# mythos-bio/mythos

Hardware: AMD Instinct MI355X
Metric: MD steps/sec (and ns/day) per GPU, oxDNA2 12 kbp duplex (higher is better)
Workload: dtype f32; 1 GPU; oxDNA2 12000 bp duplex (24000 nt), Debye-Hueckel salt 0.5, Langevin dt 0.005, free space, 1 replica/GPU; half_charged_ends=True, replicas=1, repeats=1, warmup_steps_done=10205, precision=headline f32 (north_star: fp32 at 1e-3); the other precision: --full, full=False

## Files before the change

include/mythos_hip.h:

```cpp
#ifndef MYTHOS_HIP_H
#define MYTHOS_HIP_H

#include <stdint.h>

#ifdef __cplusplus
extern "C" {
#endif

typedef struct mythos_system mythos_system_t;
typedef struct mythos_sim mythos_sim_t;
typedef struct mythos_martini mythos_martini_t;
typedef struct mythos_martini_sim mythos_martini_sim_t;
typedef struct mythos_obs mythos_obs_t;
typedef void* mythos_stream_t;

enum mythos_status {
  MYTHOS_OK = 0,
  MYTHOS_ERR_INVALID_ARGUMENT = -1,
  MYTHOS_ERR_HIP = -2,
  MYTHOS_ERR_NO_DEVICE = -3,
  MYTHOS_ERR_NOT_READY = -4,
  MYTHOS_ERR_OVERFLOW = -5,
  MYTHOS_ERR_NUMERIC = -6
};

enum mythos_dtype { MYTHOS_F32 = 0, MYTHOS_F64 = 1 };

#define MYTHOS_OXDNA_N_TERMS 8

const char* mythos_version(void);
const char* mythos_last_error(void);
int mythos_device_count(void);

int mythos_oxdna_param_count(void);
const char* mythos_oxdna_param_name(int index);

mythos_system_t* mythos_oxdna_create(int model, int n, const int32_t* seq, const uint8_t* is_end, int n_bonded,
                                     const int32_t* bonded, const double* box, int dtype, int device);
void mythos_oxdna_destroy(mythos_system_t* sys);

int mythos_oxdna_set_params(mythos_system_t* sys, const double* flat_params, int n_params);

int mythos_oxdna_set_nucleotide_types(mythos_system_t* sys, const uint8_t* is_rna);

int mythos_oxdna_set_pseq(mythos_system_t* sys, const double* marginals, const int32_t* unit, int n_bp,
                          const double* bp_probs, int terms);

int mythos_oxdna_energy_dpseq(mythos_system_t* sys, const void* center, const void* quat, int n_frames, double* e_terms,
                              void* dU_dcenter, void* dU_dquat, double* dU_dparams, double* dU_dmarginals, double* dU_dbp,
                              mythos_stream_t stream);

int mythos_oxdna_set_neighbors(mythos_system_t* sys, const int32_t* pairs, int n_pairs);

int mythos_oxdna_build_neighbors(mythos_system_t* sys, const void* center, double r_cut, double skin,
                                 mythos_stream_t stream);
int mythos_oxdna_neighbor_stats(mythos_system_t* sys, int* max_row, double* mean_row);

int mythos_oxdna_energy(mythos_system_t* sys, const void* center, const void* quat, int n_frames, double* e_terms,
                        void* dU_dcenter, void* dU_dquat, double* dU_dparams, mythos_stream_t stream);

#define MYTHOS_DEBYE_SWEEP_CONSTS 5
int mythos_oxdna_debye_sweep(mythos_system_t* sys, const void* center, const void* quat, int n_frames, int n_kt,
                             const double* dh_consts, double* e_dh, double* de_dconsts, mythos_stream_t stream);

#define MYTHOS_OP_BOND 0
#define MYTHOS_OP_MINDISTANCE 1
int mythos_oxdna_order_params(mythos_system_t* sys, const void* center, const void* quat, int n_frames, int n_ops,
                              const int32_t* op_kind, const int32_t* op_first, const int32_t* pairs, int n_pairs,
                              double hb_cutoff, double* op_out, double* hb_out, double* dist_out, mythos_stream_t stream);

mythos_obs_t* mythos_observables_create(int model, int n, const double* geometry, const double* box, int n_bp,
                                        const int32_t* base_pairs, int n_quartets, const int32_t* quartets, int skip_ends,
                                        int dtype, int device);
void mythos_observables_destroy(mythos_obs_t* obs);
int mythos_observables_width(const mythos_obs_t* obs);
int mythos_observables_eval(mythos_obs_t* obs, const void* center, const void* quat, int n_frames, double* out,
                            mythos_stream_t stream);
int mythos_oxdna_energy_obs(mythos_system_t* sys, const void* center, const void* quat, int n_frames, double* e_terms,
                            void* dU_dcenter, void* dU_dquat, double* dU_dparams, mythos_obs_t* obs, double* obs_out,
                            mythos_stream_t stream);

mythos_sim_t* mythos_langevin_create(mythos_system_t* sys, double dt, double kT, double gamma_t, double gamma_r,
                                     double mass, const double* inertia, uint64_t seed);
void mythos_langevin_destroy(mythos_sim_t* sim);

int mythos_langevin_set_neighbor_policy(mythos_sim_t* sim, double r_cut, double skin, int every);

int mythos_langevin_init_momenta(mythos_sim_t* sim, void* p_lin, void* p_ang, mythos_stream_t stream);

int mythos_langevin_run(mythos_sim_t* sim, void* center, void* quat, void* p_lin, void* p_ang, int n_steps,
                        int save_every, void* traj_center, void* traj_quat, double* e_trace,
                        mythos_stream_t stream);
int mythos_langevin_load(mythos_sim_t* sim, const void* center, const void* quat, const void* p_lin, const void* p_ang,
                         mythos_stream_t stream);
int mythos_langevin_advance(mythos_sim_t* sim, int n_steps, int save_every, void* traj_center, void* traj_quat,
                            double* e_trace, mythos_stream_t stream);
int mythos_langevin_store(mythos_sim_t* sim, void* center, void* quat, void* p_lin, void* p_ang, mythos_stream_t stream);

int64_t mythos_langevin_get_step(const mythos_sim_t* sim);
int mythos_langevin_set_step(mythos_sim_t* sim, int64_t step);
int mythos_langevin_set_seed(mythos_sim_t* sim, uint64_t seed);

int mythos_langevin_set_external_forces(mythos_sim_t* sim, int count, const int32_t* index, const double* force);

enum mythos_restraint_kind { MYTHOS_RESTRAINT_SUM = 0, MYTHOS_RESTRAINT_TORQUE = 1 };
int mythos_langevin_set_restraints(mythos_sim_t* sim, int n_tethers, const int32_t* t_index, const double* t_k, const double* t_anchor,
                                   const int32_t* t_mask, int n_groups, const int32_t* g_kind, const int32_t* g_first,
                                   const int32_t* g_member, const double* g_vec, const double* g_target, const int32_t* g_mask);

// ... 130 lines not shown
```

mythos_amd/_lib.py:

```python

from __future__ import annotations

import ctypes as C
import os
from pathlib import Path

import torch

_LIB_PATH = Path(__file__).resolve().parent / "lib" / "libmythos_hip.so"

c_int_p = C.POINTER(C.c_int32)
c_double_p = C.POINTER(C.c_double)
c_uint8_p = C.POINTER(C.c_uint8)


class MythosHipError(RuntimeError):
    """An error reported by libmythos_hip.so."""


_lib = None

V = C.c_void_p
_SIGS = {
    "mythos_version": (C.c_char_p, []),
    "mythos_last_error": (C.c_char_p, []),
    "mythos_device_count": (C.c_int, []),
    "mythos_debug_set": (C.c_int, [C.c_int, C.c_int64]),
    "mythos_debug_get": (C.c_int64, [C.c_int]),
    "mythos_oxdna_param_count": (C.c_int, []),
    "mythos_oxdna_param_name": (C.c_char_p, [C.c_int]),
    "mythos_oxdna_create": (V, [C.c_int, C.c_int, c_int_p, c_uint8_p, C.c_int, c_int_p, c_double_p, C.c_int, C.c_int]),
    "mythos_oxdna_destroy": (None, [V]),
    "mythos_oxdna_set_params": (C.c_int, [V, c_double_p, C.c_int]),
    "mythos_oxdna_set_pseq": (C.c_int, [V, c_double_p, c_int_p, C.c_int, c_double_p, C.c_int]),
    "mythos_oxdna_set_nucleotide_types": (C.c_int, [V, c_uint8_p]),
    "mythos_oxdna_set_neighbors": (C.c_int, [V, c_int_p, C.c_int]),
    "mythos_oxdna_build_neighbors": (C.c_int, [V, V, C.c_double, C.c_double, V]),
    "mythos_oxdna_neighbor_stats": (C.c_int, [V, C.POINTER(C.c_int), c_double_p]),
    "mythos_oxdna_energy": (C.c_int, [V, V, V, C.c_int, V, V, V, V, V]),
    "mythos_oxdna_energy_obs": (C.c_int, [V, V, V, C.c_int, V, V, V, V, V, V, V]),
    "mythos_oxdna_energy_dpseq": (C.c_int, [V, V, V, C.c_int, V, V, V, V, V, V, V]),
    "mythos_oxdna_debye_sweep": (C.c_int, [V, V, V, C.c_int, C.c_int, c_double_p, V, V, V]),
    "mythos_oxdna_order_params": (C.c_int, [V, V, V, C.c_int, C.c_int, c_int_p, c_int_p, c_int_p, C.c_int, C.c_double, V, V, V, V]),
    "mythos_observables_create": (V, [C.c_int, C.c_int, c_double_p, c_double_p, C.c_int, c_int_p, C.c_int, c_int_p, C.c_int, C.c_int, C.c_int]),
    "mythos_observables_destroy": (None, [V]),
    "mythos_observables_width": (C.c_int, [V]),
    "mythos_observables_eval": (C.c_int, [V, V, V, C.c_int, V, V]),
    "mythos_langevin_create": (V, [V, C.c_double, C.c_double, C.c_double, C.c_double, C.c_double, c_double_p, C.c_uint64]),
    "mythos_langevin_destroy": (None, [V]),
    "mythos_langevin_set_neighbor_policy": (C.c_int, [V, C.c_double, C.c_double, C.c_int]),
    "mythos_langevin_init_momenta": (C.c_int, [V, V, V, V]),
    "mythos_langevin_run": (C.c_int, [V, V, V, V, V, C.c_int, C.c_int, V, V, V, V]),
    "mythos_langevin_load": (C.c_int, [V, V, V, V, V, V]),
    "mythos_langevin_advance": (C.c_int, [V, C.c_int, C.c_int, V, V, V, V]),
    "mythos_langevin_store": (C.c_int, [V, V, V, V, V, V]),
    "mythos_langevin_get_step": (C.c_int64, [V]),
    "mythos_langevin_set_step": (C.c_int, [V, C.c_int64]),
    "mythos_langevin_set_seed": (C.c_int, [V, C.c_uint64]),
    "mythos_langevin_set_external_forces": (C.c_int, [V, C.c_int, c_int_p, c_double_p]),
    "mythos_langevin_set_restraints": (C.c_int, [V, C.c_int, c_int_p, c_double_p, c_double_p, c_int_p, C.c_int, c_int_p, c_int_p, c_int_p,
                                                 c_double_p, c_double_p, c_int_p]),
    "mythos_langevin_eval_external": (C.c_int, [V, V, V, V, V]),
    "mythos_langevin_set_point_forces": (C.c_int, [V, C.c_int, c_int_p, c_int_p, c_int_p, c_int_p, c_double_p]),
    "mythos_point_forces_check": (C.c_int, [C.c_int, C.c_int, C.c_int, c_int_p, c_int_p, c_int_p, c_int_p, c_double_p]),
    "mythos_langevin_eval_external_at": (C.c_int, [V, V, C.c_double, V, V, V]),
    "mythos_langevin_last_kernel_ms": (C.c_int, [V, c_double_p, c_double_p, C.POINTER(C.c_int), C.POINTER(C.c_int)]),
    "mythos_langevin_set_option": (C.c_int, [V, C.c_int, C.c_int64]),
    "mythos_langevin_set_timing": (C.c_int, [V, C.c_int]),
    "mythos_martini_langevin_set_timing": (C.c_int, [V, C.c_int]),
    "mythos_langevin_last_recoveries": (C.c_int, [V, C.POINTER(C.c_int)]),
    "mythos_langevin_last_rebuilds": (C.c_int, [V, C.POINTER(C.c_int)]),
    "mythos_oxdna_read_trajectory": (C.c_int, [C.c_char_p, C.c_int, C.c_int, c_double_p, c_double_p, c_double_p, c_double_p, C.POINTER(C.c_int)]),
    "mythos_oxdna_write_trajectory": (C.c_int, [C.c_char_p, C.c_int, C.c_int, c_double_p, c_double_p, c_double_p, c_double_p, C.c_int]),
    "mythos_martini_create": (
        V,
        [C.c_int, c_int_p, C.c_int, c_double_p, c_double_p, C.c_int, c_int_p, c_double_p, c_double_p, C.c_int,
         c_int_p, c_double_p, c_double_p, C.c_int, C.c_double, C.c_int, C.c_int],
    ),
    "mythos_martini_destroy": (None, [V]),
    "mythos_martini_energy": (C.c_int, [V, V, V, C.c_int, V, V, V]),
    "mythos_martini_param_grads": (C.c_int, [V, V, V, C.c_int, V, V, V, V, V, V, V]),
    "mythos_martini_langevin_create": (V, [V, C.c_double, C.c_double, C.c_double, c_double_p, C.c_uint64]),
    "mythos_martini_langevin_destroy": (None, [V]),
    "mythos_martini_langevin_set_neighbor_policy": (C.c_int, [V, C.c_double, C.c_int]),
    "mythos_martini_langevin_set_inner_list": (C.c_int, [V, C.c_double, C.c_int]),
    "mythos_martini_langevin_init_velocities": (C.c_int, [V, V, V]),
    "mythos_martini_langevin_run": (C.c_int, [V, V, V, c_double_p, C.c_int, C.c_int, V, V, V]),
    "mythos_martini_langevin_load": (C.c_int, [V, V, V, c_double_p, V]),
    "mythos_martini_langevin_advance": (C.c_int, [V, C.c_int, C.c_int, V, V, V]),
    "mythos_martini_langevin_store": (C.c_int, [V, V, V, V]),
    "mythos_martini_langevin_get_step": (C.c_int64, [V]),
# ... 145 lines not shown
```

mythos_amd/csrc/capi.hip:

```cpp
#include <atomic>
#include <cmath>
#include <cstring>
#include <memory>

#include "cell_list.h"
#include "observables.h"

namespace mythos {

static thread_local std::string g_last_error;

void set_error(const std::string& msg) { g_last_error = msg; }

int hip_fail(hipError_t e, const char* what) {
  g_last_error = std::string("HIP error: ") + hipGetErrorString(e) + " in " + what;
  return MYTHOS_ERR_HIP;
}

static std::atomic<long long> g_debug[MYTHOS_DEBUG_KEYS];

long long debug_value(int key) { return (key >= 0 && key < MYTHOS_DEBUG_KEYS) ? g_debug[key].load(std::memory_order_relaxed) : 0; }
void debug_clear(int key) {
  if (key >= 0 && key < MYTHOS_DEBUG_KEYS) g_debug[key].store(0, std::memory_order_relaxed);
}
// ... 207 lines not shown
      }
      double implied[4] = {0, 0, 0, 0};
      for (int t = 0; t < 4; ++t) implied[kBase[u & 1][t]] += bp_probs[4 * (size_t)(u >> 1) + t];
      for (int b = 0; b < 4; ++b)
        if (std::fabs(implied[b] - marginals[4 * (size_t)owner[u] + b]) > 1e-6) {
          set_error("mythos_oxdna_set_pseq: the marginal of nucleotide " + std::to_string(owner[u]) +
                    " is not the one its base pair's type probabilities imply");
          return MYTHOS_ERR_INVALID_ARGUMENT;
        }
    }
  }
  std::vector<double> bp(4 * (size_t)std::max(n_bp, 1), 0.0);
  if (n_bp > 0) std::copy(bp_probs, bp_probs + 4 * (size_t)n_bp, bp.begin());
  if (int rc = s->d_ps_marg.upload_real(s->dtype, marginals, 4 * (size_t)n)) return rc;
  if (int rc = s->d_ps_bp.upload_real(s->dtype, bp.data(), bp.size())) return rc;
  if (int rc = s->d_ps_unit.upload(unit, (size_t)n)) return rc;
  s->pseq_terms = terms;
  s->ps_n_bp = n_bp;
  ++s->list_epoch;
  return MYTHOS_OK;
}

int mythos_oxdna_set_neighbors(mythos_system_t* s, const int32_t* pairs, int n_pairs) {
  if (!s || n_pairs < 0 || (n_pairs > 0 && !pairs)) {
    set_error("mythos_oxdna_set_neighbors: invalid argument");
    return MYTHOS_ERR_INVALID_ARGUMENT;
  }
  MYTHOS_HIP_TRY(hipSetDevice(s->device));
  ++s->list_epoch;
  return rows_from_pairs(s, pairs, n_pairs);
}

int mythos_oxdna_build_neighbors(mythos_system_t* s, const void* center, double r_cut, double skin,
                                 mythos_stream_t stream) {
  if (!s || !center || !(r_cut > 0) || skin < 0) {
    set_error("mythos_oxdna_build_neighbors: invalid argument");
    return MYTHOS_ERR_INVALID_ARGUMENT;
  }
  MYTHOS_HIP_TRY(hipSetDevice(s->device));
  hipStream_t st = (hipStream_t)stream;
  ++s->list_epoch;
  return rows_build_until_fit(s, center, false, r_cut, skin, nullptr, nullptr, false, false, st);
}

int mythos_oxdna_neighbor_stats(mythos_system_t* s, int* max_row, double* mean_row) {
  if (!s || !s->nbrs_set) {
    set_error("mythos_oxdna_neighbor_stats: no neighbour list");
    return MYTHOS_ERR_NOT_READY;
  }
  MYTHOS_HIP_TRY(hipSetDevice(s->device));
  return row_stats(s->d_row_len.get(), s->n, ROW_BONDED_SLOTS, max_row, mean_row);
}

int mythos_oxdna_energy(mythos_system_t* s, const void* center, const void* quat, int n_frames, double* e_terms,
                        void* dU_dcenter, void* dU_dquat, double* dU_dparams, mythos_stream_t stream) {
  if (!s || n_frames < 0 || (n_frames > 0 && (!center || !quat || !e_terms))) {
    set_error("mythos_oxdna_energy: invalid argument");
    return MYTHOS_ERR_INVALID_ARGUMENT;
  }
  if (!s->params_set || !s->nbrs_set || (s->model == 4 && !s->types_set)) {
    set_error("mythos_oxdna_energy: parameters and neighbours (and, for oxNA, nucleotide types) must be set first");
    return MYTHOS_ERR_NOT_READY;
  }
  if (n_frames == 0) return MYTHOS_OK;
  MYTHOS_HIP_TRY(hipSetDevice(s->device));
  return oxdna_energy_launch(s, center, quat, n_frames, e_terms, dU_dcenter, dU_dquat, dU_dparams, nullptr, nullptr,
                             (hipStream_t)stream);
}

int mythos_oxdna_energy_dpseq(mythos_system_t* s, const void* center, const void* quat, int n_frames, double* e_terms,
                              void* dU_dcenter, void* dU_dquat, double* dU_dparams, double* dU_dmarginals, double* dU_dbp,
                              mythos_stream_t stream) {
  if (!s || n_frames < 0 || (n_frames > 0 && (!center || !quat || !e_terms || !dU_dparams || !dU_dmarginals || !dU_dbp))) {
    set_error("mythos_oxdna_energy_dpseq: invalid argument (dU_dparams and both distribution-gradient buffers are required)");
    return MYTHOS_ERR_INVALID_ARGUMENT;
  }
  if (!s->params_set || !s->nbrs_set || s->pseq_terms == 0 || (s->model == 4 && !s->types_set)) {
    set_error("mythos_oxdna_energy_dpseq: parameters, neighbours and a probabilistic sequence (mythos_oxdna_set_pseq) must be set first");
    return MYTHOS_ERR_NOT_READY;
  }
  if (n_frames == 0) return MYTHOS_OK;
  MYTHOS_HIP_TRY(hipSetDevice(s->device));
  s->ps_gmarg = dU_dmarginals, s->ps_gbp = dU_dbp;
  const int rc = oxdna_energy_launch(s, center, quat, n_frames, e_terms, dU_dcenter, dU_dquat, dU_dparams, nullptr, nullptr,
                                     (hipStream_t)stream);
  s->ps_gmarg = s->ps_gbp = nullptr;
  return rc;
}

int mythos_oxdna_energy_obs(mythos_system_t* s, const void* center, const void* quat, int n_frames, double* e_terms,
                            void* dU_dcenter, void* dU_dquat, double* dU_dparams, mythos_obs_t* obs, double* obs_out,
                            mythos_stream_t stream) {
  if (!s || n_frames < 0 || (n_frames > 0 && (!center || !quat || !e_terms)) || (obs && n_frames > 0 && !obs_out)) {
    set_error("mythos_oxdna_energy_obs: invalid argument");
    return MYTHOS_ERR_INVALID_ARGUMENT;
  }
  if (obs && (obs->n != s->n || obs->dtype != s->dtype || obs->device != s->device)) {
    set_error("mythos_oxdna_energy_obs: the observable set was made for another system size, precision or device");
    return MYTHOS_ERR_INVALID_ARGUMENT;
  }
  if (!s->params_set || !s->nbrs_set || (s->model == 4 && !s->types_set)) {
    set_error("mythos_oxdna_energy_obs: parameters and neighbours (and, for oxNA, nucleotide types) must be set first");
    return MYTHOS_ERR_NOT_READY;
  }
  if (obs && s->model == 4) {
    set_error("mythos_oxdna_energy_obs: the structural observables take one site geometry; an oxNA system has two");
// ... 10 lines not shown
```

mythos_amd/csrc/langevin_step.h:

```cpp
#pragma once
#include <hip/hip_runtime.h>

#include <cstdint>

#include "oxdna_gather.h"
#include "philox.h"

namespace mythos {

template <typename R>
struct LangevinConst {
  R dt, half_dt;
  R inv_mass;
  R inv_inertia[3];
  R c1_t, c2_t;
  R c1_r, c2_r[3];
  R skin_half_sq;
};

template <int K, typename R>
__device__ __forceinline__ void free_rotor(R* q, R* L, R h, const R* inv_I) {
  const R phi = h * L[K] * inv_I[K];
  R s, c;
  if constexpr (sizeof(R) == 4) {
// ... 267 lines not shown
                (list_overflow ? (list_overflow[0] | list_overflow[1]) : 0);
  }
  const int bid = chunk_order ? chunk_order[vb] : vb;
  const int i = bid * PPB + grp;
  const bool valid = i < n;
  const int ii = valid ? i : n - 1;

  const R g_ba = P[GEO_BASE], g_st = P[GEO_STACK];
  const CP Prna = make_cp(Pg + ((MODEL == 4) ? OXP_COUNT : 0)), Pdrh = make_cp(Pg + ((MODEL == 4) ? 2 * OXP_COUNT : 0));
  const Na1Params<CP> P4{P, Prna, Pdrh};

  Nuc<R> self;
  V3<R> offb_s, self_lo{R(0), R(0), R(0)};
  {
    const V4 s0 = in.p0[ii], s1 = in.p1[ii], s2 = in.p2[ii], s3 = in.p3[ii];
    if constexpr (kHiLo<R>) self_lo = xyz<R>(in.pl[ii]);
    self.c = xyz<R>(s0);
    self.a1 = xyz<R>(s1);
    self.a3 = xyz<R>(s2);
    self.a2 = cross(self.a3, self.a1);
    offb_s = xyz<R>(s3);
    const int m = (int)s0.w;
    self.seq = m & 3;
    self.is_end = (m >> 2) & 1;
    self.rna = (m >> 3) & 1;
    if (lane == 0) {
      R* sl = self_lds[grp];
      sl[0] = s0.x, sl[1] = s0.y, sl[2] = s0.z, sl[3] = s1.x, sl[4] = s1.y, sl[5] = s1.z;
      sl[6] = s2.x, sl[7] = s2.y, sl[8] = s2.z, sl[9] = s0.w;
      sl[10] = self_lo.x, sl[11] = self_lo.y, sl[12] = self_lo.z;
    }
  }
  const int* __restrict__ row = rows + (size_t)ii * row_stride;
  const int len = valid ? row_len[ii] : 0;
  const int close_end = min(len, row_close[ii]);

  R e[T_COUNT];
#pragma unroll
  for (int k = 0; k < T_COUNT; ++k) e[k] = R(0);
  V3<R> gbk{R(0), R(0), R(0)}, gba{R(0), R(0), R(0)};

  MD_PRIO(0);
  const RadSet<R> rs0 = (MODEL == 4) ? radset_from<R, 2>(P, cut_from<R>(P, cut.rcom2)) : radset_from<R, MODEL>(P, cut);
  const RadSet<R> rs1 = (MODEL == 4) ? radset_from<R, 2>(Prna, cut_from<R>(Prna, cut.rcom2)) : rs0;
  const RadSet<R> rs2 = (MODEL == 4) ? radset_from<R, 2>(Pdrh, cut_from<R>(Pdrh, cut.rcom2)) : rs0;
  int n_items[2] = {0, 0};
  const int row_room = ITEMS - (extra_bonds ? ROW_BONDED_SLOTS - 2 : 0);
  const int lane64 = threadIdx.x & 63;
  const int gshift = lane64 & ~(G - 1);
  auto row_at = [&](int s, int end) -> int {
    const int v = row[max(min(s, end - 1), 0)];
    return s < end ? v : -1;
  };
  auto slot_of_entry = [&](int e) -> int { return e >= 0 ? (e & ROW_INDEX_MASK) : ii; };
  {
    int e_cur = -1, e_nxt = -1;
    V4 n0{}, n3{}, n1{}, nl{};
    {
      const int s = ROW_BONDED_SLOTS + lane;
      e_cur = row_at(s, close_end);
      e_nxt = row_at(s + G, close_end);
      const int j = slot_of_entry(e_cur);
      n0 = in.p0[j];
      n3 = in.p3[j];
      n1 = in.p1[j];
      if constexpr (kHiLo<R>) nl = in.pl[j];
    }
#pragma unroll 1
    for (int s0 = ROW_BONDED_SLOTS; s0 < close_end; s0 += G) {
      const int s = s0 + lane;
      const int entry = e_cur;
      const V4 o0 = n0, o3 = n3, o1 = n1, ol = nl;
      e_cur = e_nxt;
      e_nxt = row_at(s + 2 * G, close_end);
      {
        const int jn = slot_of_entry(e_cur);
        n0 = in.p0[jn];
        n3 = in.p3[jn];
        n1 = in.p1[jn];
        if constexpr (kHiLo<R>) nl = in.pl[jn];
      }
      bool flag[2] = {false, false};
      if (entry >= 0) {
        const bool role_p = (entry & ROW_ROLE_Q) == 0;
        MD_RADSET_OF_ENTRY
        const bool o_rna = (MODEL == 4) && ((((int)o0.w) >> 3) & 1);
        const R gba_s = (MODEL == 4 && self.rna) ? Prna[GEO_BASE] : g_ba, gba_o = o_rna ? Prna[GEO_BASE] : g_ba;
        const R gst_s = (MODEL == 4 && self.rna) ? Prna[GEO_STACK] : g_st, gst_o = o_rna ? Prna[GEO_STACK] : g_st;
        (void)gst_s, (void)gst_o;
        const V3<R> dco = min_image(centre_diff<R>(o0, ol, self.c, self_lo), box);
        const V3<R> offb_o = xyz<R>(o3);
        const bool close = dot(dco, dco) < cut.rcom2;
        {
          const V3<R> d = dco + offb_o - offb_s;
          const R r2 = dot(d, d);
          if (r2 < rs.rbb2) {
            const R r = m_sqrt(r2);
            const FD<R> v = f3_eval(r, rs.eps_n, rs.f_bb);
            R dVdr = rs.tw_n * v.d;
            R en = v.f;
            if constexpr (MODEL >= 2) {
              const FD<R> dh = debye_eval(r, rs.dhp);
              R mult = R(1);
              if (rs.half_ends) {
                const int mo = (int)o0.w;
                mult = (self.is_end ? R(0.5) : R(1)) * (((mo >> 2) & 1) ? R(0.5) : R(1));
              }
              dVdr += rs.tw_dh * mult * dh.d;
              if constexpr (SAVE) e[T_DH] += R(0.5) * mult * dh.f;
            }
            if constexpr (SAVE) e[T_NEXC] += R(0.5) * en;
            axpy(gbk, dVdr / r, d);
          }
        }
        if (close) {
          const V3<R> a1o = xyz<R>(o1);
          R en = R(0);
          {
            V3<R> dA = dco - offb_s;
            axpy(dA, gba_o, a1o);
            V3<R> dB = dco + offb_o;
            axpy(dB, -gba_s, self.a1);
            const R ra2 = dot(dA, dA), rb2 = dot(dB, dB);
            R c1, c2;
            en += f3_coef(rs.eps_n, rs.tw_n, rs.f_bkba, role_p ? ra2 : rb2, c1);
            en += f3_coef(rs.eps_n, rs.tw_n, rs.f_babk, role_p ? rb2 : ra2, c2);
            axpy(gbk, role_p ? c1 : c2, dA);
            axpy(gba, role_p ? c2 : c1, dB);
          }
          const V3<R> da = a1o - self.a1;
          {
            V3<R> d = dco;
            if constexpr (MODEL == 4) {
              axpy(d, gba_o, a1o);
              axpy(d, -gba_s, self.a1);
            } else {
              axpy(d, g_ba, da);
            }
            const R r2 = dot(d, d);
            en += f3_radial(rs.eps_n, rs.tw_n, rs.f_base, d, r2, gba);
            flag[0] = rs.cr_lo2 < r2 && r2 < rs.cr_hi2;
            if (!flag[0] && rs.hb_lo2 < r2 && r2 < rs.hb_hi2) {
              const int so = (int)o0.w & 3;
              if (PSEQ && (pseq.terms & 2) != 0)
                flag[0] = rs.hb_mask != 0u;
              else
                flag[0] = (rs.hb_mask >> (role_p ? (self.seq * 4 + so) : (so * 4 + self.seq))) & 1u;
            }
          }
          {
            V3<R> d = dco;
            if constexpr (MODEL == 4) {
              axpy(d, gst_o, a1o);
              axpy(d, -gst_s, self.a1);
            } else {
              axpy(d, g_st, da);
            }
            const R r2 = dot(d, d);
            flag[1] = rs.cx_lo2 < r2 && r2 < rs.cx_hi2;
          }
          if constexpr (SAVE) e[T_NEXC] += R(0.5) * en;
        }
      }
#pragma unroll
      for (int t = 0; t < 2; ++t) {
        const unsigned long long bal = __ballot(flag[t]);
        const unsigned int gm = (unsigned int)(bal >> gshift) & ((1u << G) - 1u);
        if (flag[t]) {
          const int pos = n_items[t] + __popc(gm & ((1u << lane) - 1u));
          if (pos < ITEMS) items[t][grp][pos] = entry;
        }
        n_items[t] += __popc(gm);
      }
    }
  }
  MD_PRIO(1);
  {
    int e_cur = -1, e_nxt = -1;
    V4 n0{}, n3{}, nl{};
    {
      const int s = close_end + lane;
      e_cur = row_at(s, len);
      e_nxt = row_at(s + G, len);
      const int j = slot_of_entry(e_cur);
      n0 = in.p0[j];
      n3 = in.p3[j];
      if constexpr (kHiLo<R>) nl = in.pl[j];
    }
#pragma unroll 1
    for (int s0 = close_end; s0 < len; s0 += G) {
      const int s = s0 + lane;
      const int entry = e_cur;
      const V4 o0 = n0, o3 = n3, ol = nl;
      e_cur = e_nxt;
      e_nxt = row_at(s + 2 * G, len);
      {
        const int jn = slot_of_entry(e_cur);
        n0 = in.p0[jn];
        n3 = in.p3[jn];
        if constexpr (kHiLo<R>) nl = in.pl[jn];
      }
      if (entry >= 0) {
        MD_RADSET_OF_ENTRY
        const V3<R> dco = min_image(centre_diff<R>(o0, ol, self.c, self_lo), box);
        const V3<R> d = dco + xyz<R>(o3) - offb_s;
        const R r2 = dot(d, d);
        if (r2 < rs.rbb2) {
          const R r = m_sqrt(r2);
          const FD<R> v = f3_eval(r, rs.eps_n, rs.f_bb);
          R dVdr = rs.tw_n * v.d;
          if constexpr (MODEL >= 2) {
            const FD<R> dh = debye_eval(r, rs.dhp);
            R mult = R(1);
            if (rs.half_ends) {
              const int mo = (int)o0.w;
              mult = (self.is_end ? R(0.5) : R(1)) * (((mo >> 2) & 1) ? R(0.5) : R(1));
            }
            dVdr += rs.tw_dh * mult * dh.d;
            if constexpr (SAVE) e[T_DH] += R(0.5) * mult * dh.f;
          }
          if constexpr (SAVE) e[T_NEXC] += R(0.5) * v.f;
          axpy(gbk, dVdr / r, d);
        }
      }
    }
  }
  if (n_items[0] + n_items[1] > row_room) {
    if (lane == 0) atomicMax(flags + 3, k_index + 1);
    n_items[0] = n_items[1] = 0;
  }
  group_reduce_v3<G>(gbk);
  group_reduce_v3<G>(gba);
  if (lane == 0) {
    R* rl = rad_lds[grp];
    rl[0] = gbk.x, rl[1] = gbk.y, rl[2] = gbk.z, rl[3] = gba.x, rl[4] = gba.y, rl[5] = gba.z;
#pragma unroll
    for (int t = 0; t < 2; ++t) item_cnt[t][grp] = valid ? n_items[t] : 0;
  }
  if (threadIdx.x == 0) s_halt = halt_word;
  __syncthreads();
  MD_PRIO(2);
  if (s_halt != 0) return;
  if (vb == 0 && threadIdx.x == 0) flags[2] = k_index + 1;

  {
    NoPG pg;
    const int wave = ((threadIdx.x >> 6) + bid) & 3;
    const bool bonded_wave = wave == 0;
    const int lst = wave == 3 ? 1 : 0;
    const int pw = threadIdx.x >> 6;
    const int n_bonded_rows = extra_bonds ? ROW_BONDED_SLOTS : 2;
    {
      const int l = threadIdx.x & 63;
      int inc = (l < PPB) ? item_cnt[lst][l] : 0;
      int rows_inc = (kPooled && l < PPB) ? n_bonded_rows + item_cnt[0][l] + item_cnt[1][l] : 0;
#pragma unroll
      for (int o = 1; o < PPB; o <<= 1) {
        const int u = __shfl_up(inc, o, 64);
        if (l >= o) inc += u;
        if constexpr (kPooled) {
          const int v = __shfl_up(rows_inc, o, 64);
          if (l >= o) rows_inc += v;
        }
      }
      if (l < PPB) item_pre[pw][l + 1] = inc;
      if (l == 0) item_pre[pw][0] = 0;
      if constexpr (kPooled) {
        if (l < PPB) row_base[pw][l + 1] = rows_inc;
        if (l == 0) row_base[pw][0] = 0;
      }
      __builtin_amdgcn_wave_barrier();
      __builtin_amdgcn_fence(__ATOMIC_ACQ_REL, "wavefront");
    }
    const bool pool_over = kPooled && row_base[kPooled ? pw : 0][PPB] > kPool;
    if (pool_over && threadIdx.x == 0) atomicMax(flags + 3, k_index + 1);
// ... 291 lines not shown
```

mythos_amd/hip_system.py:

```python

from __future__ import annotations

import ctypes as C

import numpy as np
import torch

from mythos_amd import _lib

N_TERMS = 8
TRACE_WIDTH = 10
TERM_NAMES = (
    "fene",
    "bonded_excluded_volume",
    "stacking",
    "unbonded_excluded_volume",
    "hydrogen_bonding",
    "cross_stacking",
    "coaxial_stacking",
    "debye",
)


class OxdnaSystem(_lib.Handle):
# ... 33 lines not shown
        if self.model == 4:
            if is_rna is None:
                raise ValueError("an oxNA system (model 4) needs is_rna, the type of every nucleotide")
            t = np.ascontiguousarray(is_rna, dtype=np.uint8)
            if t.shape != (self.n,):
                raise ValueError(f"is_rna must have shape ({self.n},)")
            _lib.check(self._lib.mythos_oxdna_set_nucleotide_types(self._h, t.ctypes.data_as(_lib.c_uint8_p)), "set_nucleotide_types")

    def set_params(self, flat) -> None:
        flat = np.ascontiguousarray(torch.as_tensor(flat).detach().cpu().numpy(), dtype=np.float64)
        _lib.check(
            self._lib.mythos_oxdna_set_params(self._h, flat.ctypes.data_as(_lib.c_double_p), int(flat.shape[0])),
            "set_params",
        )

    def set_pseq(self, marginals=None, unit=None, bp_probs=None, terms: int = 0) -> None:
        if not terms:
            _lib.check(self._lib.mythos_oxdna_set_pseq(self._h, None, None, 0, None, 0), "set_pseq")
            self._pseq_terms = 0
            return
        marg = np.ascontiguousarray(marginals, dtype=np.float64)
        unit = np.ascontiguousarray(unit, dtype=np.int32)
        bp = np.ascontiguousarray(bp_probs, dtype=np.float64).reshape(-1, 4)
        if marg.shape != (self.n, 4) or unit.shape != (self.n,):
            raise ValueError(f"marginals must be ({self.n}, 4) and unit ({self.n},)")
        n_bp = int(bp.shape[0]) if (unit >= 0).any() else 0
        self._pseq_n_bp = n_bp
        if (unit >= 0).any() and int(unit.max()) >= 2 * n_bp:
            raise ValueError("bp_probs has fewer rows than the base pairs named in unit")
        _lib.check(self._lib.mythos_oxdna_set_pseq(self._h, marg.ctypes.data_as(_lib.c_double_p), unit.ctypes.data_as(_lib.c_int_p),
                                                   n_bp, bp.ctypes.data_as(_lib.c_double_p), int(terms)), "set_pseq")
        self._pseq_terms = int(terms)

    def set_neighbors(self, pairs) -> None:
        pairs = np.ascontiguousarray(pairs, dtype=np.int32)
        if pairs.ndim != 2 or (pairs.size and pairs.shape[1] != 2):
            raise ValueError("pairs must have shape (P, 2)")
        _lib.check(
            self._lib.mythos_oxdna_set_neighbors(self._h, pairs.ctypes.data_as(_lib.c_int_p), int(pairs.shape[0])),
            "set_neighbors",
        )

    def build_neighbors(self, center: torch.Tensor, r_cut: float, skin: float) -> None:
        c = self._check(center, (self.n, 3), "center")
        _lib.check(
            self._lib.mythos_oxdna_build_neighbors(self._h, _lib.ptr(c), float(r_cut), float(skin), _lib.stream(self.device)),
            "build_neighbors",
        )

    def neighbor_stats(self) -> tuple[int, float]:
        mx, mean = C.c_int(0), C.c_double(0.0)
        _lib.check(self._lib.mythos_oxdna_neighbor_stats(self._h, C.byref(mx), C.byref(mean)), "neighbor_stats")
        return mx.value, mean.value

    def _check(self, t: torch.Tensor, tail: tuple, name: str) -> torch.Tensor:
        if not isinstance(t, torch.Tensor) or t.device != self.device:
            raise ValueError(f"{name} must be a torch tensor on {self.device}")
        if t.dtype != self.dtype:
            raise ValueError(f"{name} must have dtype {self.dtype}, got {t.dtype}")
        if tuple(t.shape[-len(tail):]) != tail:
            raise ValueError(f"{name} must have trailing shape {tail}, got {tuple(t.shape)}")
        return t.contiguous()

    def _frames(self, center, quat):
        single = center.dim() == 2
        c = self._check(center, (self.n, 3), "center")
        q = self._check(quat, (self.n, 4), "quat")
        if single:
            c, q = c[None], q[None]
        if q.shape[0] != c.shape[0]:
            raise ValueError("center and quat disagree on the number of frames")
        return c, q, int(c.shape[0]), single

    def energy(self, center, quat, *, grads=False, param_grads=False, observables=None, pseq_grads=False):
        c, q, nf, single = self._frames(center, quat)
        e = torch.empty((nf, N_TERMS), dtype=torch.float64, device=self.device)
        gc = torch.empty_like(c) if grads else None
        gq = torch.empty_like(q) if grads else None
        gp = torch.empty((nf, self.n_params), dtype=torch.float64, device=self.device) if param_grads else None
        if pseq_grads:
            if not param_grads or observables is not None:
                raise ValueError("pseq_grads comes with param_grads and without fused observables")
            gm = torch.empty((nf, self.n, 4), dtype=torch.float64, device=self.device)
            gb = torch.empty((nf, max(self._pseq_n_bp, 1), 4), dtype=torch.float64, device=self.device)
            _lib.check(
                self._lib.mythos_oxdna_energy_dpseq(
                    self._h, _lib.ptr(c), _lib.ptr(q), nf, _lib.ptr(e), _lib.ptr(gc), _lib.ptr(gq), _lib.ptr(gp), _lib.ptr(gm),
                    _lib.ptr(gb), _lib.stream(self.device),
                ),
                "energy_dpseq",
            )
            if single:
                return e[0], (gc[0] if grads else None), (gq[0] if grads else None), gp[0], gm[0], gb[0]
            return e, gc, gq, gp, gm, gb
        if observables is not None and not getattr(observables, "fusable", True):
            raise ValueError(f"{type(observables).__name__} is not evaluated in the energy call (the fused energy + observables "
                             "path takes an ObservableSet of propeller twist / rise / pitch / persistence length)")
        if observables is None:
            _lib.check(
                self._lib.mythos_oxdna_energy(
                    self._h, _lib.ptr(c), _lib.ptr(q), nf, _lib.ptr(e), _lib.ptr(gc), _lib.ptr(gq), _lib.ptr(gp),
                    _lib.stream(self.device),
                ),
                "energy",
            )
            rows = None
# ... 449 lines not shown
```

Before: 69840 steps/s.

## Merge close and far neighbour loops into one wavefront-uniform loop in MD kernel

```diff
diff --git a/include/mythos_hip.h b/include/mythos_hip.h
--- a/include/mythos_hip.h
+++ b/include/mythos_hip.h
@@ -55,6 +55,7 @@
 int mythos_oxdna_build_neighbors(mythos_system_t* sys, const void* center, double r_cut, double skin,
                                  mythos_stream_t stream);
 int mythos_oxdna_neighbor_stats(mythos_system_t* sys, int* max_row, double* mean_row);
+int mythos_oxdna_get_rows(mythos_system_t* sys, int32_t* rows, int32_t* row_len, int32_t* row_close, int* stride);
 
 int mythos_oxdna_energy(mythos_system_t* sys, const void* center, const void* quat, int n_frames, double* e_terms,
                         void* dU_dcenter, void* dU_dquat, double* dU_dparams, mythos_stream_t stream);
diff --git a/mythos_amd/_lib.py b/mythos_amd/_lib.py
--- a/mythos_amd/_lib.py
+++ b/mythos_amd/_lib.py
@@ -37,6 +37,7 @@
     "mythos_oxdna_set_neighbors": (C.c_int, [V, c_int_p, C.c_int]),
     "mythos_oxdna_build_neighbors": (C.c_int, [V, V, C.c_double, C.c_double, V]),
     "mythos_oxdna_neighbor_stats": (C.c_int, [V, C.POINTER(C.c_int), c_double_p]),
+    "mythos_oxdna_get_rows": (C.c_int, [V, C.POINTER(C.c_int32), C.POINTER(C.c_int32), C.POINTER(C.c_int32), C.POINTER(C.c_int)]),
     "mythos_oxdna_energy": (C.c_int, [V, V, V, C.c_int, V, V, V, V, V]),
     "mythos_oxdna_energy_obs": (C.c_int, [V, V, V, C.c_int, V, V, V, V, V, V, V]),
     "mythos_oxdna_energy_dpseq": (C.c_int, [V, V, V, C.c_int, V, V, V, V, V, V, V]),
diff --git a/mythos_amd/csrc/capi.hip b/mythos_amd/csrc/capi.hip
--- a/mythos_amd/csrc/capi.hip
+++ b/mythos_amd/csrc/capi.hip
@@ -283,6 +283,26 @@
   return row_stats(s->d_row_len.get(), s->n, ROW_BONDED_SLOTS, max_row, mean_row);
 }
 
+int mythos_oxdna_get_rows(mythos_system_t* s, int32_t* rows, int32_t* row_len, int32_t* row_close, int* stride) {
+  if (!s) {
+    set_error("mythos_oxdna_get_rows: invalid argument");
+    return MYTHOS_ERR_INVALID_ARGUMENT;
+  }
+  if (!s->nbrs_set) {
+    set_error("mythos_oxdna_get_rows: no neighbour list");
+    return MYTHOS_ERR_NOT_READY;
+  }
+  if (stride) *stride = s->list.stride;
+  if (!rows && !row_len && !row_close) return MYTHOS_OK;
+  MYTHOS_HIP_TRY(hipSetDevice(s->device));
+  MYTHOS_HIP_TRY(hipDeviceSynchronize());
+  const size_t n = (size_t)s->n;
+  if (rows) MYTHOS_HIP_TRY(hipMemcpy(rows, s->list.d_rows.get(), n * s->list.stride * sizeof(int), hipMemcpyDeviceToHost));
+  if (row_len) MYTHOS_HIP_TRY(hipMemcpy(row_len, s->d_row_len.get(), n * sizeof(int), hipMemcpyDeviceToHost));
+  if (row_close) MYTHOS_HIP_TRY(hipMemcpy(row_close, row_close_of(s), n * sizeof(int), hipMemcpyDeviceToHost));
+  return MYTHOS_OK;
+}
+
 int mythos_oxdna_energy(mythos_system_t* s, const void* center, const void* quat, int n_frames, double* e_terms,
                         void* dU_dcenter, void* dU_dquat, double* dU_dparams, mythos_stream_t stream) {
   if (!s || n_frames < 0 || (n_frames > 0 && (!center || !quat || !e_terms))) {
diff --git a/mythos_amd/csrc/langevin_step.h b/mythos_amd/csrc/langevin_step.h
--- a/mythos_amd/csrc/langevin_step.h
+++ b/mythos_amd/csrc/langevin_step.h
@@ -343,53 +343,165 @@
     const int v = row[max(min(s, end - 1), 0)];
     return s < end ? v : -1;
   };
+  auto row_word = [&](int s) -> int { return row[max(min(s, len - 1), 0)]; };
   auto slot_of_entry = [&](int e) -> int { return e >= 0 ? (e & ROW_INDEX_MASK) : ii; };
-  {
-    int e_cur = -1, e_nxt = -1;
-    V4 n0{}, n3{}, n1{}, nl{};
+  if constexpr (MODEL == 4 || GL != kMdG) {
     {
-      const int s = ROW_BONDED_SLOTS + lane;
-      e_cur = row_at(s, close_end);
-      e_nxt = row_at(s + G, close_end);
-      const int j = slot_of_entry(e_cur);
-      n0 = in.p0[j];
-      n3 = in.p3[j];
-      n1 = in.p1[j];
-      if constexpr (kHiLo<R>) nl = in.pl[j];
-    }
+      int e_cur = -1, e_nxt = -1;
+      V4 n0{}, n3{}, n1{}, nl{};
+      {
+        const int s = ROW_BONDED_SLOTS + lane;
+        e_cur = row_at(s, close_end);
+        e_nxt = row_at(s + G, close_end);
+        const int j = slot_of_entry(e_cur);
+        n0 = in.p0[j];
+        n3 = in.p3[j];
+        n1 = in.p1[j];
+        if constexpr (kHiLo<R>) nl = in.pl[j];
+      }
 #pragma unroll 1
-    for (int s0 = ROW_BONDED_SLOTS; s0 < close_end; s0 += G) {
-      const int s = s0 + lane;
-      const int entry = e_cur;
-      const V4 o0 = n0, o3 = n3, o1 = n1, ol = nl;
-      e_cur = e_nxt;
-      e_nxt = row_at(s + 2 * G, close_end);
+      for (int s0 = ROW_BONDED_SLOTS; s0 < close_end; s0 += G) {
+        const int s = s0 + lane;
+        const int entry = e_cur;
+        const V4 o0 = n0, o3 = n3, o1 = n1, ol = nl;
+        e_cur = e_nxt;
+        e_nxt = row_at(s + 2 * G, close_end);
+        {
+          const int jn = slot_of_entry(e_cur);
+          n0 = in.p0[jn];
+          n3 = in.p3[jn];
+          n1 = in.p1[jn];
+          if constexpr (kHiLo<R>) nl = in.pl[jn];
+        }
+        bool flag[2] = {false, false};
+        if (entry >= 0) {
+          const bool role_p = (entry & ROW_ROLE_Q) == 0;
+          MD_RADSET_OF_ENTRY
+          const bool o_rna = (MODEL == 4) && ((((int)o0.w) >> 3) & 1);
+          const R gba_s = (MODEL == 4 && self.rna) ? Prna[GEO_BASE] : g_ba, gba_o = o_rna ? Prna[GEO_BASE] : g_ba;
+          const R gst_s = (MODEL == 4 && self.rna) ? Prna[GEO_STACK] : g_st, gst_o = o_rna ? Prna[GEO_STACK] : g_st;
+          (void)gst_s, (void)gst_o;
+          const V3<R> dco = min_image(centre_diff<R>(o0, ol, self.c, self_lo), box);
+          const V3<R> offb_o = xyz<R>(o3);
+          const bool close = dot(dco, dco) < cut.rcom2;
+          {
+            const V3<R> d = dco + offb_o - offb_s;
+            const R r2 = dot(d, d);
+            if (r2 < rs.rbb2) {
+              const R r = m_sqrt(r2);
+              const FD<R> v = f3_eval(r, rs.eps_n, rs.f_bb);
+              R dVdr = rs.tw_n * v.d;
+              R en = v.f;
+              if constexpr (MODEL >= 2) {
+                const FD<R> dh = debye_eval(r, rs.dhp);
+                R mult = R(1);
+                if (rs.half_ends) {
+                  const int mo = (int)o0.w;
+                  mult = (self.is_end ? R(0.5) : R(1)) * (((mo >> 2) & 1) ? R(0.5) : R(1));
+                }
+                dVdr += rs.tw_dh * mult * dh.d;
+                if constexpr (SAVE) e[T_DH] += R(0.5) * mult * dh.f;
+              }
+              if constexpr (SAVE) e[T_NEXC] += R(0.5) * en;
+              axpy(gbk, dVdr / r, d);
+            }
+          }
+          if (close) {
+            const V3<R> a1o = xyz<R>(o1);
+            R en = R(0);
+            {
+              V3<R> dA = dco - offb_s;
+              axpy(dA, gba_o, a1o);
+              V3<R> dB = dco + offb_o;
+              axpy(dB, -gba_s, self.a1);
+              const R ra2 = dot(dA, dA), rb2 = dot(dB, dB);
+              R c1, c2;
+              en += f3_coef(rs.eps_n, rs.tw_n, rs.f_bkba, role_p ? ra2 : rb2, c1);
+              en += f3_coef(rs.eps_n, rs.tw_n, rs.f_babk, role_p ? rb2 : ra2, c2);
+              axpy(gbk, role_p ? c1 : c2, dA);
+              axpy(gba, role_p ? c2 : c1, dB);
+            }
+            const V3<R> da = a1o - self.a1;
+            {
+              V3<R> d = dco;
+              if constexpr (MODEL == 4) {
+                axpy(d, gba_o, a1o);
+                axpy(d, -gba_s, self.a1);
+              } else {
+                axpy(d, g_ba, da);
+              }
+              const R r2 = dot(d, d);
+              en += f3_radial(rs.eps_n, rs.tw_n, rs.f_base, d, r2, gba);
+              flag[0] = rs.cr_lo2 < r2 && r2 < rs.cr_hi2;
+              if (!flag[0] && rs.hb_lo2 < r2 && r2 < rs.hb_hi2) {
+                const int so = (int)o0.w & 3;
+                if (PSEQ && (pseq.terms & 2) != 0)
+                  flag[0] = rs.hb_mask != 0u;
+                else
+                  flag[0] = (rs.hb_mask >> (role_p ? (self.seq * 4 + so) : (so * 4 + self.seq))) & 1u;
+              }
+            }
+            {
+              V3<R> d = dco;
+              if constexpr (MODEL == 4) {
+                axpy(d, gst_o, a1o);
+                axpy(d, -gst_s, self.a1);
+              } else {
+                axpy(d, g_st, da);
+              }
+              const R r2 = dot(d, d);
+              flag[1] = rs.cx_lo2 < r2 && r2 < rs.cx_hi2;
+            }
+            if constexpr (SAVE) e[T_NEXC] += R(0.5) * en;
+          }
+        }
+#pragma unroll
+        for (int t = 0; t < 2; ++t) {
+          const unsigned long long bal = __ballot(flag[t]);
+          const unsigned int gm = (unsigned int)(bal >> gshift) & ((1u << G) - 1u);
+          if (flag[t]) {
+            const int pos = n_items[t] + __popc(gm & ((1u << lane) - 1u));
+            if (pos < ITEMS) items[t][grp][pos] = entry;
+          }
+          n_items[t] += __popc(gm);
+        }
+      }
+    }
+    MD_PRIO(1);
+    {
+      int e_cur = -1, e_nxt = -1;
+      V4 n0{}, n3{}, nl{};
       {
-        const int jn = slot_of_entry(e_cur);
-        n0 = in.p0[jn];
-        n3 = in.p3[jn];
-        n1 = in.p1[jn];
-        if constexpr (kHiLo<R>) nl = in.pl[jn];
-      }
-      bool flag[2] = {false, false};
-      if (entry >= 0) {
-        const bool role_p = (entry & ROW_ROLE_Q) == 0;
-        MD_RADSET_OF_ENTRY
-        const bool o_rna = (MODEL == 4) && ((((int)o0.w) >> 3) & 1);
-        const R gba_s = (MODEL == 4 && self.rna) ? Prna[GEO_BASE] : g_ba, gba_o = o_rna ? Prna[GEO_BASE] : g_ba;
-        const R gst_s = (MODEL == 4 && self.rna) ? Prna[GEO_STACK] : g_st, gst_o = o_rna ? Prna[GEO_STACK] : g_st;
-        (void)gst_s, (void)gst_o;
-        const V3<R> dco = min_image(centre_diff<R>(o0, ol, self.c, self_lo), box);
-        const V3<R> offb_o = xyz<R>(o3);
-        const bool close = dot(dco, dco) < cut.rcom2;
+        const int s = close_end + lane;
+        e_cur = row_at(s, len);
+        e_nxt = row_at(s + G, len);
+        const int j = slot_of_entry(e_cur);
+        n0 = in.p0[j];
+        n3 = in.p3[j];
+        if constexpr (kHiLo<R>) nl = in.pl[j];
+      }
+#pragma unroll 1
+      for (int s0 = close_end; s0 < len; s0 += G) {
+        const int s = s0 + lane;
+        const int entry = e_cur;
+        const V4 o0 = n0, o3 = n3, ol = nl;
+        e_cur = e_nxt;
+        e_nxt = row_at(s + 2 * G, len);
         {
-          const V3<R> d = dco + offb_o - offb_s;
+          const int jn = slot_of_entry(e_cur);
+          n0 = in.p0[jn];
+          n3 = in.p3[jn];
+          if constexpr (kHiLo<R>) nl = in.pl[jn];
+        }
+        if (entry >= 0) {
+          MD_RADSET_OF_ENTRY
+          const V3<R> dco = min_image(centre_diff<R>(o0, ol, self.c, self_lo), box);
+          const V3<R> d = dco + xyz<R>(o3) - offb_s;
           const R r2 = dot(d, d);
           if (r2 < rs.rbb2) {
             const R r = m_sqrt(r2);
             const FD<R> v = f3_eval(r, rs.eps_n, rs.f_bb);
             R dVdr = rs.tw_n * v.d;
-            R en = v.f;
             if constexpr (MODEL >= 2) {
               const FD<R> dh = debye_eval(r, rs.dhp);
               R mult = R(1);
@@ -400,118 +512,165 @@
               dVdr += rs.tw_dh * mult * dh.d;
               if constexpr (SAVE) e[T_DH] += R(0.5) * mult * dh.f;
             }
-            if constexpr (SAVE) e[T_NEXC] += R(0.5) * en;
+            if constexpr (SAVE) e[T_NEXC] += R(0.5) * v.f;
             axpy(gbk, dVdr / r, d);
           }
         }
-        if (close) {
-          const V3<R> a1o = xyz<R>(o1);
-          R en = R(0);
-          {
-            V3<R> dA = dco - offb_s;
-            axpy(dA, gba_o, a1o);
-            V3<R> dB = dco + offb_o;
-            axpy(dB, -gba_s, self.a1);
-            const R ra2 = dot(dA, dA), rb2 = dot(dB, dB);
-            R c1, c2;
-            en += f3_coef(rs.eps_n, rs.tw_n, rs.f_bkba, role_p ? ra2 : rb2, c1);
-            en += f3_coef(rs.eps_n, rs.tw_n, rs.f_babk, role_p ? rb2 : ra2, c2);
-            axpy(gbk, role_p ? c1 : c2, dA);
-            axpy(gba, role_p ? c2 : c1, dB);
-          }
-          const V3<R> da = a1o - self.a1;
-          {
-            V3<R> d = dco;
-            if constexpr (MODEL == 4) {
-              axpy(d, gba_o, a1o);
-              axpy(d, -gba_s, self.a1);
-            } else {
-              axpy(d, g_ba, da);
+      }
+    }
+  } else {
+    {
+      int e_cur = -1, e_nxt = -1;
+      V4 n0{}, n3{}, n1{}, nl{};
+      int wlen = 0, wclose = 0;
+#pragma unroll
+      for (int k = 0; k < 64 / G; ++k) {
+        wlen = max(wlen, __builtin_amdgcn_readlane(len, k * G));
+        wclose = max(wclose, __builtin_amdgcn_readlane(close_end, k * G));
+      }
+      int s0 = ROW_BONDED_SLOTS;
+      if (s0 < wlen) {
+        const int s = s0 + lane;
+        e_cur = row_at(s, len);
+        if (s0 + G < wlen) e_nxt = row_word(s + G);
+        const int j = slot_of_entry(e_cur);
+        n0 = in.p0[j];
+        n3 = in.p3[j];
+        if (s0 < wclose) n1 = in.p1[j];
+        if constexpr (kHiLo<R>) nl = in.pl[j];
+      }
+#pragma unroll 1
+      for (; s0 < wlen; s0 += G) {
+        const int s = s0 + lane;
+        const int entry = e_cur;
+        const V4 o0 = n0, o3 = n3, o1 = n1, ol = nl;
+        e_cur = s + G < len ? e_nxt : -1;
+        if (s0 + G < wlen) {
+          if (s0 + 2 * G < wlen) e_nxt = row_word(s + 2 * G);
+          const int jn = slot_of_entry(e_cur);
+          n0 = in.p0[jn];
+          n3 = in.p3[jn];
+          if (s0 + G < wclose) n1 = in.p1[jn];
+          if constexpr (kHiLo<R>) nl = in.pl[jn];
+        }
+        if (s0 < wclose) {
+          bool flag[2] = {false, false};
+          if (entry >= 0) {
+            const bool role_p = (entry & ROW_ROLE_Q) == 0;
+            MD_RADSET_OF_ENTRY
+            const bool o_rna = (MODEL == 4) && ((((int)o0.w) >> 3) & 1);
+            const R gba_s = (MODEL == 4 && self.rna) ? Prna[GEO_BASE] : g_ba, gba_o = o_rna ? Prna[GEO_BASE] : g_ba;
+            const R gst_s = (MODEL == 4 && self.rna) ? Prna[GEO_STACK] : g_st, gst_o = o_rna ? Prna[GEO_STACK] : g_st;
+            (void)gst_s, (void)gst_o;
+            const V3<R> dco = min_image(centre_diff<R>(o0, ol, self.c, self_lo), box);
+            const V3<R> offb_o = xyz<R>(o3);
+            const bool close = s < close_end && dot(dco, dco) < cut.rcom2;
+            {
+              const V3<R> d = dco + offb_o - offb_s;
+              const R r2 = dot(d, d);
+              if (r2 < rs.rbb2) {
+                const R r = m_sqrt(r2);
+                const FD<R> v = f3_eval(r, rs.eps_n, rs.f_bb);
+                R dVdr = rs.tw_n * v.d;
+                R en = v.f;
+                if constexpr (MODEL >= 2) {
+                  const FD<R> dh = debye_eval(r, rs.dhp);
+                  R mult = R(1);
+                  if (rs.half_ends) {
+                    const int mo = (int)o0.w;
+                    mult = (self.is_end ? R(0.5) : R(1)) * (((mo >> 2) & 1) ? R(0.5) : R(1));
+                  }
+                  dVdr += rs.tw_dh * mult * dh.d;
+                  if constexpr (SAVE) e[T_DH] += R(0.5) * mult * dh.f;
+                }
+                if constexpr (SAVE) e[T_NEXC] += R(0.5) * en;
+                axpy(gbk, dVdr / r, d);
+              }
             }
-            const R r2 = dot(d, d);
-            en += f3_radial(rs.eps_n, rs.tw_n, rs.f_base, d, r2, gba);
-            flag[0] = rs.cr_lo2 < r2 && r2 < rs.cr_hi2;
-            if (!flag[0] && rs.hb_lo2 < r2 && r2 < rs.hb_hi2) {
-              const int so = (int)o0.w & 3;
-              if (PSEQ && (pseq.terms & 2) != 0)
-                flag[0] = rs.hb_mask != 0u;
-              else
-                flag[0] = (rs.hb_mask >> (role_p ? (self.seq * 4 + so) : (so * 4 + self.seq))) & 1u;
+            if (close) {
+              const V3<R> a1o = xyz<R>(o1);
+              R en = R(0);
+              {
+                V3<R> dA = dco - offb_s;
+                axpy(dA, gba_o, a1o);
+                V3<R> dB = dco + offb_o;
+                axpy(dB, -gba_s, self.a1);
+                const R ra2 = dot(dA, dA), rb2 = dot(dB, dB);
+                R c1, c2;
+                en += f3_coef(rs.eps_n, rs.tw_n, rs.f_bkba, role_p ? ra2 : rb2, c1);
+                en += f3_coef(rs.eps_n, rs.tw_n, rs.f_babk, role_p ? rb2 : ra2, c2);
+                axpy(gbk, role_p ? c1 : c2, dA);
+                axpy(gba, role_p ? c2 : c1, dB);
+              }
+              const V3<R> da = a1o - self.a1;
+              {
+                V3<R> d = dco;
+                if constexpr (MODEL == 4) {
+                  axpy(d, gba_o, a1o);
+                  axpy(d, -gba_s, self.a1);
+                } else {
+                  axpy(d, g_ba, da);
+                }
+                const R r2 = dot(d, d);
+                en += f3_radial(rs.eps_n, rs.tw_n, rs.f_base, d, r2, gba);
+                flag[0] = rs.cr_lo2 < r2 && r2 < rs.cr_hi2;
+                if (!flag[0] && rs.hb_lo2 < r2 && r2 < rs.hb_hi2) {
+                  const int so = (int)o0.w & 3;
+                  if (PSEQ && (pseq.terms & 2) != 0)
+                    flag[0] = rs.hb_mask != 0u;
+                  else
+                    flag[0] = (rs.hb_mask >> (role_p ? (self.seq * 4 + so) : (so * 4 + self.seq))) & 1u;
+                }
+              }
+              {
+                V3<R> d = dco;
+                if constexpr (MODEL == 4) {
+                  axpy(d, gst_o, a1o);
+                  axpy(d, -gst_s, self.a1);
+                } else {
+                  axpy(d, g_st, da);
+                }
+                const R r2 = dot(d, d);
+                flag[1] = rs.cx_lo2 < r2 && r2 < rs.cx_hi2;
+              }
+              if constexpr (SAVE) e[T_NEXC] += R(0.5) * en;
             }
           }
-          {
-            V3<R> d = dco;
-            if constexpr (MODEL == 4) {
-              axpy(d, gst_o, a1o);
-              axpy(d, -gst_s, self.a1);
-            } else {
-              axpy(d, g_st, da);
+#pragma unroll
+          for (int t = 0; t < 2; ++t) {
+            const unsigned long long bal = __ballot(flag[t]);
+            const unsigned int gm = (unsigned int)(bal >> gshift) & ((1u << G) - 1u);
+            if (flag[t]) {
+              const int pos = n_items[t] + __popc(gm & ((1u << lane) - 1u));
+              if (pos < ITEMS) items[t][grp][pos] = entry;
             }
+            n_items[t] += __popc(gm);
+          }
+        } else {
+          MD_PRIO(1);
+          if (entry >= 0) {
+            MD_RADSET_OF_ENTRY
+            const V3<R> dco = min_image(centre_diff<R>(o0, ol, self.c, self_lo), box);
+            const V3<R> d = dco + xyz<R>(o3) - offb_s;
             const R r2 = dot(d, d);
-            flag[1] = rs.cx_lo2 < r2 && r2 < rs.cx_hi2;
+            if (r2 < rs.rbb2) {
+              const R r = m_sqrt(r2);
+              const FD<R> v = f3_eval(r, rs.eps_n, rs.f_bb);
+              R dVdr = rs.tw_n * v.d;
+              if constexpr (MODEL >= 2) {
+                const FD<R> dh = debye_eval(r, rs.dhp);
+                R mult = R(1);
+                if (rs.half_ends) {
+                  const int mo = (int)o0.w;
+                  mult = (self.is_end ? R(0.5) : R(1)) * (((mo >> 2) & 1) ? R(0.5) : R(1));
+                }
+                dVdr += rs.tw_dh * mult * dh.d;
+                if constexpr (SAVE) e[T_DH] += R(0.5) * mult * dh.f;
+              }
+              if constexpr (SAVE) e[T_NEXC] += R(0.5) * v.f;
+              axpy(gbk, dVdr / r, d);
+            }
           }
-          if constexpr (SAVE) e[T_NEXC] += R(0.5) * en;
-        }
-      }
-#pragma unroll
-      for (int t = 0; t < 2; ++t) {
-        const unsigned long long bal = __ballot(flag[t]);
-        const unsigned int gm = (unsigned int)(bal >> gshift) & ((1u << G) - 1u);
-        if (flag[t]) {
-          const int pos = n_items[t] + __popc(gm & ((1u << lane) - 1u));
-          if (pos < ITEMS) items[t][grp][pos] = entry;
-        }
-        n_items[t] += __popc(gm);
-      }
-    }
-  }
-  MD_PRIO(1);
-  {
-    int e_cur = -1, e_nxt = -1;
-    V4 n0{}, n3{}, nl{};
-    {
-      const int s = close_end + lane;
-      e_cur = row_at(s, len);
-      e_nxt = row_at(s + G, len);
-      const int j = slot_of_entry(e_cur);
-      n0 = in.p0[j];
-      n3 = in.p3[j];
-      if constexpr (kHiLo<R>) nl = in.pl[j];
-    }
-#pragma unroll 1
-    for (int s0 = close_end; s0 < len; s0 += G) {
-      const int s = s0 + lane;
-      const int entry = e_cur;
-      const V4 o0 = n0, o3 = n3, ol = nl;
-      e_cur = e_nxt;
-      e_nxt = row_at(s + 2 * G, len);
-      {
-        const int jn = slot_of_entry(e_cur);
-        n0 = in.p0[jn];
-        n3 = in.p3[jn];
-        if constexpr (kHiLo<R>) nl = in.pl[jn];
-      }
-      if (entry >= 0) {
-        MD_RADSET_OF_ENTRY
-        const V3<R> dco = min_image(centre_diff<R>(o0, ol, self.c, self_lo), box);
-        const V3<R> d = dco + xyz<R>(o3) - offb_s;
-        const R r2 = dot(d, d);
-        if (r2 < rs.rbb2) {
-          const R r = m_sqrt(r2);
-          const FD<R> v = f3_eval(r, rs.eps_n, rs.f_bb);
-          R dVdr = rs.tw_n * v.d;
-          if constexpr (MODEL >= 2) {
-            const FD<R> dh = debye_eval(r, rs.dhp);
-            R mult = R(1);
-            if (rs.half_ends) {
-              const int mo = (int)o0.w;
-              mult = (self.is_end ? R(0.5) : R(1)) * (((mo >> 2) & 1) ? R(0.5) : R(1));
-            }
-            dVdr += rs.tw_dh * mult * dh.d;
-            if constexpr (SAVE) e[T_DH] += R(0.5) * mult * dh.f;
-          }
-          if constexpr (SAVE) e[T_NEXC] += R(0.5) * v.f;
-          axpy(gbk, dVdr / r, d);
         }
       }
     }
diff --git a/mythos_amd/hip_system.py b/mythos_amd/hip_system.py
--- a/mythos_amd/hip_system.py
+++ b/mythos_amd/hip_system.py
@@ -109,6 +109,17 @@
         mx, mean = C.c_int(0), C.c_double(0.0)
         _lib.check(self._lib.mythos_oxdna_neighbor_stats(self._h, C.byref(mx), C.byref(mean)), "neighbor_stats")
         return mx.value, mean.value
+
+    def rows(self):
+        stride = C.c_int(0)
+        _lib.check(self._lib.mythos_oxdna_get_rows(self._h, None, None, None, C.byref(stride)), "get_rows")
+        rows = np.empty((self.n, stride.value), dtype=np.int32)
+        lens = np.empty(self.n, dtype=np.int32)
+        close = np.empty(self.n, dtype=np.int32)
+        p32 = C.POINTER(C.c_int32)
+        _lib.check(self._lib.mythos_oxdna_get_rows(self._h, rows.ctypes.data_as(p32), lens.ctypes.data_as(p32),
+                                                   close.ctypes.data_as(p32), C.byref(stride)), "get_rows")
+        return rows, lens, close
 
     def _check(self, t: torch.Tensor, tail: tuple, name: str) -> torch.Tensor:
         if not isinstance(t, torch.Tensor) or t.device != self.device:
```

Result: faster. 70590 steps/s (median of 6 runs) (+1.1%).
